# BrunoudA/MH-PPO

Measured on AMD Instinct MI355X. Metric: env-steps/sec at 65536 envs × 4 agents, 1/2/4/8 MI355X + %HBM roofline, higher is better.
Workload: dtype f64 env / f32 nets; 1 GPU; config 3: 4cars nb_car=4 nb_ped=1 nb_lines=2, 65536 envs/GPU x 80 steps, full PPO iteration (rollout + returns + 10+10 epochs); envs_per_gpu=65536, agents=4, T=80, parallelism=dp1

## Files before the change

### include/mhppo.h

```cpp
#ifndef MHPPO_H
#define MHPPO_H
#include <stdint.h>

#ifdef __cplusplus
extern "C" {
#endif

#define MHPPO_OK 0
#define MHPPO_EINVAL -1
#define MHPPO_EHIP -2
#define MHPPO_ENOMEM -3
#define MHPPO_ENAN -4

#define MHPPO_COOP 0
#define MHPPO_4CARS 1
#define MHPPO_SCALABLE 2
#define MHPPO_NAIF 3
#define MHPPO_4CARS2 4
#define MHPPO_STOP 5
#define MHPPO_FIX_SCALABLE_LANES 1
#define MHPPO_GENERIC_STEP 2

typedef struct mhppo_env_cfg {
    int32_t variant;
// ... 91 lines not shown
int mhppo_rollout_policy(mhppo_env *env, const mhppo_mlp *actor_cross, const mhppo_mlp *actor_wait,
                         mhppo_rollout_bufs *bufs, void *stream);
int mhppo_rollout_sample_env(mhppo_env *env, const float *eps, int t, mhppo_rollout_bufs *bufs, void *stream);
int mhppo_rollout_policy_part(mhppo_env *env, const mhppo_mlp *actor_cross, const mhppo_mlp *actor_wait,
                              mhppo_rollout_bufs *bufs, int part, void *stream);
int mhppo_rollout_sample_env_part(mhppo_env *env, const float *eps, int t, mhppo_rollout_bufs *bufs, int part,
                                  void *stream);

int mhppo_kernel_timing_begin(int n);
int mhppo_kernel_timing_end(double *ms_total, int *launches);
int mhppo_kernel_timing_end_each(float *ms_each, int cap, int *launches);

int mhppo_rollout_check(mhppo_rollout_bufs *bufs, void *stream);

int mhppo_philox_normal(uint64_t seed, uint64_t offset, float *out, int64_t n, void *stream);
int mhppo_philox_uniform(uint64_t seed, uint64_t offset, float *out, int64_t n, void *stream);
int mhppo_philox_normal_2d(uint64_t seed, uint64_t offset, uint64_t stride, float *out, int64_t rows,
                           int64_t cols, void *stream);


int mhppo_libm_eval(int fn, uint64_t first, int64_t n, float *out, void *stream);

int mhppo_returns_scan(const double *rew, float *ret, int64_t B, int32_t T, double gamma, void *stream);
int mhppo_returns_scan_tm(const double *rew, float *ret, int64_t B, int32_t T, double gamma, void *stream);

typedef struct {
  float *obs, *act, *logp, *ret;
  double *rew;
} mhppo_bucket_dst;
int mhppo_bucket_scatter(const int64_t *pos, const int8_t *bucket, int64_t NS, int32_t T, const float *obs_tm,
                         const float *act_tm, const float *logp_tm, const float *ret_tm, const double *rew_tm,
                         const mhppo_bucket_dst *dst, void *stream);

int mhppo_adv_stats(const float *ret, const float *value, int64_t M, double *stats, void *stream);
int mhppo_adv_normalize(const float *ret, const float *value, int64_t M, const double *stats,
                        double m_global, float *adv, void *stream);

int mhppo_ppo_cont_fwd_bwd(const float *mu, const float *act, const float *logp_old,
                           const float *adv, int64_t M, double inv_m, float *dmu,
                           double *loss, void *stream);

int mhppo_ppo_choice_fwd_bwd(const float *probs, const float *logp_old, const float *adv,
                             int64_t M, const double *counts, double inv_m2, float *dprobs,
                             double *loss, void *stream);

#define MHPPO_TRAIN_EXACT_F32 0x100
int mhppo_mlp_train(int kind, int n_in, const float *packed, const float *X, int64_t M, const float *ret,
                    float *value, const float *act, const float *logp_old, const double *stats,
                    const double *counts, double m_global, float out_mean, float out_std, float *grad,
                    double *sums, void *stream);

int mhppo_mlp_train_pair(const float *packed_actor, const float *packed_critic, const float *X, int64_t M,
                         const float *ret, float *value, const float *act, const float *logp_old,
                         const double *stats, double m_global, float out_mean, float out_std,
                         float *grad_actor, double *sums_actor, float *grad_critic, double *sums_critic,
                         void *stream);

int mhppo_mse_fwd_bwd(const float *value, const float *ret, int64_t M, double inv_m, float *dv,
                      double *loss, void *stream);

const char *mhppo_last_error(void);
const char *mhppo_version(void);

#ifdef __cplusplus
}
#endif
// ... 2 lines not shown
```

### mh-ppo_amd/csrc/rollout.hip

```cpp
#include <hip/hip_runtime.h>
#include <hip/hip_ext.h>

#include <vector>

#include <algorithm>
#include <math.h>
#include <string.h>

#include "../../include/mhppo.h"
#include "common.h"
#include "env_body.h"
#include "rollout_dev.h"
#include "libm_glibc.h"

using namespace mhppo;

namespace mhppo {
const Cfg &env_cfg(const mhppo_env *env);
const Bufs &env_bufs(const mhppo_env *env);
int env_device(const mhppo_env *env);
}

namespace {
constexpr int TPB = 256;
// ... 745 lines not shown
__global__ void __launch_bounds__(TPB) k_philox_normal_2d(uint64_t seed, uint64_t off, uint64_t stride, float *out,
                                                          int64_t rows, int64_t cols) {
  const int64_t i = (int64_t)blockIdx.x * TPB + threadIdx.x;
  if (i >= rows * cols) return;
  const int64_t r = i / cols, cc = i - r * cols;
  const uint64_t ctr = off + (uint64_t)r * stride + (uint64_t)cc;
  uint32_t c4[4] = {(uint32_t)ctr, (uint32_t)(ctr >> 32), 0x6d687070u, 0u};
  philox(c4, (uint32_t)seed, (uint32_t)(seed >> 32));
  const float u1 = ((float)(c4[0] >> 8) + 1.0f) * (1.0f / 16777216.0f);
  const float u2 = (float)(c4[1] >> 8) * (1.0f / 16777216.0f);
  out[i] = sqrtf(-2.0f * logf(u1)) * cosf(6.2831853071795865f * u2);
}

__global__ void __launch_bounds__(TPB) k_returns(const double *rew, float *ret, int64_t B, int T, double gamma) {
  int64_t b = (int64_t)blockIdx.x * TPB + threadIdx.x;
  if (b >= B) return;
  const double *r = rew + b * T;
  float *o = ret + b * T;
  double g = 0.0;
  for (int t = T - 1; t >= 0; t--) {
    g = r[t] + gamma * g;
    o[t] = (float)g;
  }
}

namespace bk {
constexpr int SEGS = 64, STEPS = 16;
constexpr int OBS_SEG = STEPS * NF_C + 1, V_SEG = STEPS + 1;
#ifndef MHPPO_BK_TPB
#define MHPPO_BK_TPB 1024
#endif
constexpr int BTPB = MHPPO_BK_TPB;
}
__global__ void __launch_bounds__(bk::BTPB)
    k_bucket_scatter(const int64_t *__restrict__ pos, const int8_t *__restrict__ bucket, int64_t NS, int T,
                     const float *__restrict__ obs, const float *__restrict__ act, const float *__restrict__ logp,
                     const float *__restrict__ ret, const double *__restrict__ rew, mhppo_bucket_dst d0,
                     mhppo_bucket_dst d1) {
  using namespace bk;
  __shared__ float s_obs[SEGS * OBS_SEG];
  __shared__ float s_v[3][SEGS * V_SEG];
  __shared__ double s_rew[SEGS * V_SEG];
  __shared__ int64_t s_pos[SEGS];
  __shared__ int8_t s_b[SEGS];
  const int64_t s0 = (int64_t)blockIdx.x * SEGS;
  const int t0 = blockIdx.y * STEPS;
  const int nseg = (int)min((int64_t)SEGS, NS - s0), nt = min(STEPS, T - t0);
  const int tid = threadIdx.x;
  if (tid < SEGS) {
    s_pos[tid] = tid < nseg ? pos[s0 + tid] : -1;
    s_b[tid] = tid < nseg ? bucket[s0 + tid] : 0;
  }
  __syncthreads();
  {
    constexpr int NQ = SEGS * NF_C * STEPS / BTPB;
    static_assert(SEGS * NF_C * STEPS % BTPB == 0, "bucket scatter: block size");
    float v[NQ];
    int at[NQ];
#pragma unroll
    for (int q = 0; q < NQ; q++) {
      const int i = tid + q * BTPB, tl = i / (SEGS * NF_C), k = i - tl * (SEGS * NF_C), sg = k / NF_C;
      const bool in = sg < nseg && tl < nt;
      at[q] = in && s_pos[sg] >= 0 ? sg * OBS_SEG + tl * NF_C + (k - sg * NF_C) : -1;
      v[q] = 0.0f;
      if (at[q] >= 0) v[q] = obs[((int64_t)(t0 + tl) * NS + s0) * NF_C + k];
    }
#pragma unroll
    for (int q = 0; q < NQ; q++)
      if (at[q] >= 0) s_obs[at[q]] = v[q];
  }
#pragma unroll
  for (int i = tid; i < SEGS * STEPS; i += BTPB) {
    const int sg = i % SEGS, tl = i / SEGS;
    if (sg >= nseg || tl >= nt || s_pos[sg] < 0) continue;
    const int64_t rec = (int64_t)(t0 + tl) * NS + s0 + sg;
    const int o = sg * V_SEG + tl;
    s_v[0][o] = act[rec];
    s_v[1][o] = logp[rec];
    s_v[2][o] = ret[rec];
    s_rew[o] = rew[rec];
  }
  __syncthreads();
  const int w = tid >> 6, l = tid & 63;
  for (int sg = w; sg < nseg; sg += BTPB / 64) {
    const int64_t p = s_pos[sg];
    if (p < 0) continue;
    const mhppo_bucket_dst &D = s_b[sg] ? d1 : d0;
    const int64_t r0 = p * T + t0;
    float *oo = D.obs + r0 * NF_C;
    for (int j = l; j < nt * NF_C; j += 64) oo[j] = s_obs[sg * OBS_SEG + j];
    if (l < nt) {
      const int o = sg * V_SEG + l;
      D.act[r0 + l] = s_v[0][o];
      D.logp[r0 + l] = s_v[1][o];
      D.ret[r0 + l] = s_v[2][o];
      D.rew[r0 + l] = s_rew[o];
    }
  }
}

__global__ void __launch_bounds__(TPB) k_returns_tm(const double *rew, float *ret, int64_t B, int T, double gamma) {
  int64_t b = (int64_t)blockIdx.x * TPB + threadIdx.x;
  if (b >= B) return;
  double g = 0.0;
  for (int t = T - 1; t >= 0; t--) {
    g = rew[(int64_t)t * B + b] + gamma * g;
    ret[(int64_t)t * B + b] = (float)g;
  }
}

template <int NP>
__device__ inline void block_reduce_store(double (&v)[NP], double *partials, int nblocks) {
  __shared__ double sh[NP][TPB];
#pragma unroll
  for (int k = 0; k < NP; k++) sh[k][threadIdx.x] = v[k];
  __syncthreads();
  for (int s = TPB / 2; s > 0; s >>= 1) {
    if ((int)threadIdx.x < s)
#pragma unroll
      for (int k = 0; k < NP; k++) sh[k][threadIdx.x] += sh[k][threadIdx.x + s];
    __syncthreads();
  }
  if (threadIdx.x == 0)
#pragma unroll
    for (int k = 0; k < NP; k++) partials[(size_t)k * nblocks + blockIdx.x] = sh[k][0];
}

__global__ void __launch_bounds__(TPB) k_sum_partials(const double *partials, int nblocks, int np, double *out) {
  __shared__ double sh[TPB];
  int k = blockIdx.x;
  double s = 0.0;
  for (int b = threadIdx.x; b < nblocks; b += TPB) s += partials[(size_t)k * nblocks + b];
  sh[threadIdx.x] = s;
  __syncthreads();
  for (int w = TPB / 2; w > 0; w >>= 1) {
    if ((int)threadIdx.x < w) sh[threadIdx.x] += sh[threadIdx.x + w];
    __syncthreads();
  }
  if (threadIdx.x == 0) out[k] += sh[0];
}

__global__ void __launch_bounds__(TPB) k_adv_stats(const float *ret, const float *val, int64_t M, double *partials) {
  int64_t i = (int64_t)blockIdx.x * TPB + threadIdx.x;
  double v[2] = {0.0, 0.0};
  if (i < M) {
    float a = ret[i] - val[i];
    v[0] = a;
    v[1] = (double)a * (double)a;
  }
  block_reduce_store<2>(v, partials, gridDim.x);
}

__global__ void __launch_bounds__(TPB)
    k_adv_norm(const float *ret, const float *val, int64_t M, const double *stats, double mg, float *adv) {
  int64_t i = (int64_t)blockIdx.x * TPB + threadIdx.x;
  if (i >= M) return;
  double mean = stats[0] / mg;
  double var = (stats[1] - stats[0] * mean) / (mg - 1.0);
  float meanf = (float)mean, stdf = (float)sqrt(var > 0 ? var : 0.0);
  float a = ret[i] - val[i];
  adv[i] = (a - meanf) / (stdf + 1e-10f);
}

__global__ void __launch_bounds__(TPB)
    k_ppo_cont(const float *mu, const float *act, const float *lp_old, const float *adv, int64_t M, double inv_m,
               float *dmu, double *partials) {
  int64_t i = (int64_t)blockIdx.x * TPB + threadIdx.x;
  double v[1] = {0.0};
  if (i < M) {
    float diff = (float)((double)act[i] - (double)mu[i]);
    float x = diff * MVN_INV_L;
    float lp = (-0.5f * (MVN_LOG2PI + x * x)) - MVN_HALF_LOGDET;
// ... 444 lines not shown
  if (!out || n < 0 || fn < 0 || fn > 2) return set_error(MHPPO_EINVAL, "bad argument (fn 0 tanhf, 1 expm1f, 2 expf)");
  if (n == 0) return MHPPO_OK;
  hipLaunchKernelGGL(k_libm_eval, grid_for(n), dim3(TPB), 0, (hipStream_t)stream, fn, first, n, out);
  CHECK_HIP(hipGetLastError());
  return MHPPO_OK;
}

int mhppo_returns_scan(const double *rew, float *ret, int64_t B, int32_t T, double gamma, void *stream) {
  if (!rew || !ret || B < 0 || T <= 0) return set_error(MHPPO_EINVAL, "bad argument");
  if (B == 0) return MHPPO_OK;
  hipLaunchKernelGGL(k_returns, grid_for(B), dim3(TPB), 0, (hipStream_t)stream, rew, ret, B, T, gamma);
  CHECK_HIP(hipGetLastError());
  return MHPPO_OK;
}

int mhppo_returns_scan_tm(const double *rew, float *ret, int64_t B, int32_t T, double gamma, void *stream) {
  if (!rew || !ret || B < 0 || T <= 0) return set_error(MHPPO_EINVAL, "bad argument");
  if (B == 0) return MHPPO_OK;
  hipLaunchKernelGGL(k_returns_tm, grid_for(B), dim3(TPB), 0, (hipStream_t)stream, rew, ret, B, T, gamma);
  CHECK_HIP(hipGetLastError());
  return MHPPO_OK;
}

int mhppo_bucket_scatter(const int64_t *pos, const int8_t *bucket, int64_t NS, int32_t T, const float *obs_tm,
                         const float *act_tm, const float *logp_tm, const float *ret_tm, const double *rew_tm,
                         const mhppo_bucket_dst *dst, void *stream) {
  if (NS < 0 || T <= 0 || !dst) return set_error(MHPPO_EINVAL, "bad argument");
  if (NS == 0) return MHPPO_OK;
  if (!pos || !bucket || !obs_tm || !act_tm || !logp_tm || !ret_tm || !rew_tm)
    return set_error(MHPPO_EINVAL, "null pointer");
  const int64_t nb = (NS + bk::SEGS - 1) / bk::SEGS;
  if (nb > 0x7fffffff) return set_error(MHPPO_EINVAL, "too many segments");
  dim3 g((unsigned)nb, (unsigned)((T + bk::STEPS - 1) / bk::STEPS));
  hipLaunchKernelGGL(k_bucket_scatter, g, dim3(bk::BTPB), 0, (hipStream_t)stream, pos, bucket, NS, (int)T, obs_tm,
                     act_tm, logp_tm, ret_tm, rew_tm, dst[0], dst[1]);
  CHECK_HIP(hipGetLastError());
  return MHPPO_OK;
}

int mhppo_adv_stats(const float *ret, const float *value, int64_t M, double *stats, void *stream) {
  if (M == 0) return MHPPO_OK;
  if (!ret || !value || !stats || M < 0) return set_error(MHPPO_EINVAL, "bad argument");
  dim3 g = grid_for(M);
  double *part = scratch(2 * (size_t)g.x);
  if (!part) return set_error(MHPPO_ENOMEM, "scratch allocation failed");
  hipStream_t s = (hipStream_t)stream;
  hipLaunchKernelGGL(k_adv_stats, g, dim3(TPB), 0, s, ret, value, M, part);
  hipLaunchKernelGGL(k_sum_partials, dim3(2), dim3(TPB), 0, s, part, (int)g.x, 2, stats);
  CHECK_HIP(hipGetLastError());
  return MHPPO_OK;
}

int mhppo_adv_normalize(const float *ret, const float *value, int64_t M, const double *stats, double m_global,
                        float *adv, void *stream) {
  if (M == 0) return MHPPO_OK;
  if (!ret || !value || !stats || !adv || M < 0) return set_error(MHPPO_EINVAL, "bad argument");
  hipLaunchKernelGGL(k_adv_norm, grid_for(M), dim3(TPB), 0, (hipStream_t)stream, ret, value, M, stats, m_global,
                     adv);
  CHECK_HIP(hipGetLastError());
  return MHPPO_OK;
}

int mhppo_ppo_cont_fwd_bwd(const float *mu, const float *act, const float *logp_old, const float *adv, int64_t M,
                           double inv_m, float *dmu, double *loss, void *stream) {
  if (M == 0) return MHPPO_OK;
  if (!mu || !act || !logp_old || !adv || !dmu || !loss || M < 0) return set_error(MHPPO_EINVAL, "bad argument");
  dim3 g = grid_for(M);
  double *part = scratch(g.x);
// ... 39 lines not shown
```

### mh-ppo_amd/mhppo/_lib.py

```python
import ctypes
import os

HERE = os.path.dirname(os.path.abspath(__file__))
LIB_PATH = os.environ.get("MHPPO_LIB") or os.path.join(HERE, "lib", "libmhppo.so")

P = ctypes.c_void_p
I32 = ctypes.c_int32
I64 = ctypes.c_int64
U64 = ctypes.c_uint64
F64 = ctypes.c_double


class EnvCfg(ctypes.Structure):
    _fields_ = [
        ("variant", I32), ("n_envs", I32), ("nb_car", I32), ("nb_ped", I32), ("nb_lines", I32),
        ("max_episode", I32), ("sin_model", I32), ("flags", I32), ("dt", F64),
        ("car_b", F64 * 4), ("ped_b", F64 * 8), ("cross_b", F64 * 2), ("seed_base", U64),
        ("env_id_offset", U64),
    ]


class Mlp(ctypes.Structure):
    _fields_ = [("packed", P), ("n_in", I32), ("n_out", I32), ("kind", I32), ("reserved", I32),
                ("mean", ctypes.c_float), ("std", ctypes.c_float)]
# ... 23 lines not shown
    "mhppo_env_reward_slots": (I32, [P]),
    "mhppo_env_state_dim": (I32, [P]),
    "mhppo_env_reset": (I32, [P, P, P]),
    "mhppo_env_choix_test": (I32, [P, P, P]),
    "mhppo_env_state_bytes": (I64, [P]),
    "mhppo_env_export": (I32, [P, P, P]),
    "mhppo_env_import": (I32, [P, P, P]),
    "mhppo_env_step": (I32, [P, P, P, P, P, P, P]),
    "mhppo_env_get_state": (I32, [P, P, P]),
    "mhppo_env_get_rng": (I32, [P, P, P, P]),
    "mhppo_env_events": (I32, [P, P, P]),
    "mhppo_choice_dim": (I32, [P]),
    "mhppo_rollout_begin": (I32, [P, ctypes.POINTER(Mlp), P, P, ctypes.POINTER(RolloutBufs), P]),
    "mhppo_rollout_step": (I32, [P, ctypes.POINTER(Mlp), ctypes.POINTER(Mlp), P, I32,
                                 ctypes.POINTER(RolloutBufs), P]),
    "mhppo_rollout_policy": (I32, [P, ctypes.POINTER(Mlp), ctypes.POINTER(Mlp), ctypes.POINTER(RolloutBufs), P]),
    "mhppo_rollout_sample_env": (I32, [P, P, I32, ctypes.POINTER(RolloutBufs), P]),
    "mhppo_rollout_policy_part": (I32, [P, ctypes.POINTER(Mlp), ctypes.POINTER(Mlp), ctypes.POINTER(RolloutBufs), I32,
                                        P]),
    "mhppo_rollout_sample_env_part": (I32, [P, P, I32, ctypes.POINTER(RolloutBufs), I32, P]),
    "mhppo_kernel_timing_begin": (I32, [I32]),
    "mhppo_kernel_timing_end": (I32, [ctypes.POINTER(ctypes.c_double), ctypes.POINTER(I32)]),
    "mhppo_kernel_timing_end_each": (I32, [P, I32, ctypes.POINTER(I32)]),
    "mhppo_eval_step": (I32, [P, ctypes.POINTER(Mlp), ctypes.POINTER(Mlp), ctypes.POINTER(Mlp), I32,
                              ctypes.POINTER(EvalBufs), P]),
    "mhppo_rollout_check": (I32, [ctypes.POINTER(RolloutBufs), P]),
    "mhppo_philox_normal": (I32, [U64, U64, P, I64, P]),
    "mhppo_philox_uniform": (I32, [U64, U64, P, I64, P]),
    "mhppo_philox_normal_2d": (I32, [U64, U64, U64, P, I64, I64, P]),
    "mhppo_libm_eval": (I32, [I32, U64, I64, P, P]),
    "mhppo_returns_scan": (I32, [P, P, I64, I32, F64, P]),
    "mhppo_returns_scan_tm": (I32, [P, P, I64, I32, F64, P]),
    "mhppo_bucket_scatter": (I32, [P, P, I64, I32] + [P] * 7),
    "mhppo_adv_stats": (I32, [P, P, I64, P, P]),
    "mhppo_adv_normalize": (I32, [P, P, I64, P, F64, P, P]),
    "mhppo_ppo_cont_fwd_bwd": (I32, [P, P, P, P, I64, F64, P, P, P]),
    "mhppo_ppo_choice_fwd_bwd": (I32, [P, P, P, I64, P, F64, P, P, P]),
    "mhppo_mse_fwd_bwd": (I32, [P, P, I64, F64, P, P, P]),
    "mhppo_mlp_train": (I32, [I32, I32, P, P, I64, P, P, P, P, P, P, F64, ctypes.c_float, ctypes.c_float, P, P, P]),
    "mhppo_mlp_train_pair": (I32, [P, P, P, I64, P, P, P, P, P, F64, ctypes.c_float, ctypes.c_float, P, P, P, P, P]),
    "mhppo_last_error": (ctypes.c_char_p, []),
    "mhppo_version": (ctypes.c_char_p, []),
}

_lib = None


class MhppoError(RuntimeError):
    pass


class MhppoNaNError(MhppoError, ValueError):
    """MHPPO_ENAN: a NaN policy output was sampled (the reference raises ValueError there)."""

ENAN = -4


def lib():
    global _lib
    if _lib is None:
        if not os.path.exists(LIB_PATH):
            raise MhppoError(f"{LIB_PATH} is missing: build it with `python -c 'import __graft_entry__ as g; g.build()'`")
        L = ctypes.CDLL(LIB_PATH)
        for name, (res, args) in _SIGS.items():
            fn = getattr(L, name)
            fn.restype = res
# ... 27 lines not shown
```

### mh-ppo_amd/mhppo/algo.py

```python
import contextlib
import os

import numpy as np
import torch
import torch.distributed as dist

from . import _lib, ppo
from .env import VecCrosswalk
from .models import Model_PPO
from .rollout import RolloutGPU, bucket_segments

PREFIX = {"scalable": "pappo-scalable-coop", "coop": "pappo-coop", "4cars": "pappo-coop-4cars", "naif": "pappo-acc6"}


def _rank():
    return dist.get_rank() if dist.is_available() and dist.is_initialized() else 0


def _rank_path(path):
    if dist.is_available() and dist.is_initialized() and dist.get_world_size() > 1:
        return f"{path}.rank{dist.get_rank()}"
    return path


# ... 163 lines not shown
            if m_d > 0:
                heads.append(ppo.Head("d", self.actor_net_choice, self.critic_net_choice, self.optimizer_actor_choice,
                                      self.optimizer_critic_choice, d["obs"], d["act"], d["logp"], d["ret"], m_d,
                                      counts, per_row=self.fix_choice_loss, exact=self.exact_f32))
                names.append("choice")
            losses = ppo.train_epochs(heads, 10, self.grad_bucket) if heads else None
        if self.verbose and losses is not None:
            div = {"cross": (m_c, m_c), "wait": (m_w, m_w), "choice": (m_d * m_d, m_d)}
            if self.fix_choice_loss:
                div["choice"] = (m_d, m_d)
            self.last_losses = {k: (float(a.item()) / div[k][0], float(b.item()) / div[k][1])
                                for k, (a, b) in zip(names, losses)}
        return m_c, m_w, m_d

    def evaluate(self, nbr_episodes, choix=False):
        self.rollout.reset()
        return self.rollout.iterations(self.actor_net_cross, self.actor_net_wait, self.actor_net_choice,
                                       nbr_episodes, choix=choix)

    def get_average(self, states):
        from .stats import get_average
        v = self.venv
        return get_average(states, v.variant, v.nb_car, v.nb_ped, v.nb_lines)

    def train(self, nb_loop, replay=None):
        self.rollout.fix_bucket = self.fix_bucket
        for ep in range(nb_loop):
            self.rollout.reset()
            fc, et = replay[ep] if replay is not None else (None, None)
            self.rollout.iterations_rand(self.actor_net_cross, self.actor_net_wait, self.actor_net_choice,
                                         self.cov_mat, self.cov_mat_d, self.batch_size, forced_choice=fc,
                                         eps_tape=et)
            m_c, m_w, m_d = self.update()
            rc, rw, rd = self.rollout.immediate_rewards()
            dev = self.venv.device
            sums = torch.stack([rc.double().sum(), rw.double().sum(), rd.double().sum()]).to(dev)
            ppo._allreduce_(sums)
            if dev.type == "cuda":
                host = torch.empty(3, dtype=torch.float64, pin_memory=True)
                host.copy_(sums, non_blocking=True)
                ev = torch.cuda.Event()
                ev.record(torch.cuda.current_stream(dev))
                self._pending_curves.append((host, ev, m_c, m_w, m_d))
            else:
                self._pending_curves.append((sums.clone(), None, m_c, m_w, m_d))
            if self.verbose:
                self._flush_curves()
            if self.verbose and _rank() == 0:
                print("Episode * {} * And Number of steps is ==> {}".format(ep, ep * self.batch_size))
                print("Average Cross reward is ==> {}, Average Wait reward is ==> {}".format(
                    np.mean(self.ep_reward_cross[-10:]) if self.ep_reward_cross else float("nan"),
                    np.mean(self.ep_reward_wait[-10:]) if self.ep_reward_wait else float("nan")))
                print("Average Choice reward is ==> {}".format(np.mean(self.ep_reward_choice[-10:])))
                print("Number Cross is ==> {} and Number Wait is ==> {} ".format(int(m_c), int(m_w)))
            self.rollout.reset()
            self.total_loop = self.total_loop + 1
            if len(self._pending_curves) > 1:
                self._flush_curves(keep_last=True)
        self._flush_curves()
        if _rank() == 0 and self.save_curves:
            self.save_reward_curves()
        if self.verbose and _rank() == 0:
            print("Complete")

    def _flush_curves(self, keep_last=False):
        n = len(self._pending_curves) - (1 if keep_last else 0)
        for host, ev, m_c, m_w, m_d in self._pending_curves[:n]:
            if ev is not None:
                ev.synchronize()
# ... 91 lines not shown
```

### mh-ppo_amd/mhppo/ppo.py

```python
import contextlib
import os

import torch
import torch.distributed as dist

from . import _lib


_FORCE_COLLECTIVES = False


def set_force_collectives(flag=True):
    global _FORCE_COLLECTIVES
    _FORCE_COLLECTIVES = bool(flag)


def _dp():
    if not (dist.is_available() and dist.is_initialized()):
        return False
    return _FORCE_COLLECTIVES or dist.get_world_size() > 1


def _allreduce_(t):
    if _dp():
# ... 293 lines not shown
def _actor_pass(p, h, stats, sums, st):
    ev = _ev_begin()
    _lib.check(_lib.lib().mhppo_mlp_train(
        p.akind | p.flags, p.n_in, p.wa, p.obs.data_ptr(), p.M, p.ret.data_ptr(), p.V.data_ptr(),
        None if p.act is None else p.act.data_ptr(), p.lp.data_ptr(), stats.data_ptr(),
        None if p.counts is None else p.counts.data_ptr(), h.m, p.mean, p.std, p.ga, sums.data_ptr(), st))
    _ev_end(ev, p.akind, p.n_in, p.M)


def _pair_pass(p, h, stats, sums_a, sums_c, st):
    ev = _ev_begin()
    _lib.check(_lib.lib().mhppo_mlp_train_pair(
        p.wa, p.wc, p.obs.data_ptr(), p.M, p.ret.data_ptr(), p.V.data_ptr(), p.act.data_ptr(), p.lp.data_ptr(),
        stats.data_ptr(), h.m, p.mean, p.std, p.ga, sums_a.data_ptr(), p.gc, sums_c.data_ptr(), st))
    _ev_end(ev, 3, 13, p.M)


TRAIN_STREAMS = max(1, int(os.environ.get("MHPPO_TRAIN_STREAMS", "1")))
_SIDE_STREAMS = {}


def _side_streams(dev, n):
    if dev.type != "cuda" or n <= 0:
        return []
    key = (dev.index if dev.index is not None else torch.cuda.current_device(), n)
    if key not in _SIDE_STREAMS:
        _SIDE_STREAMS[key] = [torch.cuda.Stream(device=dev) for _ in range(n)]
    return _SIDE_STREAMS[key]


def train_epochs(heads, n_epochs, bucket=None):
    H = len(heads)
    dev = heads[0].obs.device
    paired = [_use_pair(h) for h in heads]
    plans = [_HeadPlan(h) if h.obs.shape[0] > 0 else None for h in heads]
    main = torch.cuda.current_stream(dev) if dev.type == "cuda" else None
    side = _side_streams(dev, min(TRAIN_STREAMS, H) - 1)
    streams = [main] + side
    stats = None
    out = [[None, None] for _ in range(H)]
    for k in range(n_epochs + 1):
        sums = torch.zeros(2 * H, 3, dtype=torch.float64, device=dev)
        crit = k < n_epochs
        trained = []
        if side:
            fork = torch.cuda.Event()
            fork.record(main)
            for sd in side:
                sd.wait_event(fork)
        for i, h in enumerate(heads):
            p = plans[i]
            sc, sa = sums[i], sums[H + i]
            sti = streams[i % len(streams)]
            ctx = torch.cuda.stream(sti) if sti is not None else contextlib.nullcontext()
            st = sti.cuda_stream if sti is not None else None
            with ctx:
                stp = stats[2 * i:2 * i + 2] if k > 0 else None
                if p is None:
                    if k > 0:
                        cont = h.kind == "c"
                        k_mlp_train(KIND_CONT if cont else KIND_CHOICE, h.actor, h.obs, h.ret, h.obs.new_empty(0),
                                    h.act if (cont or h.per_row) else None, h.logp, stp,
                                    None if (cont or h.per_row) else h.counts, m_global=h.m, sums=sa, exact=h.exact)
                        trained.append(h.actor)
                        out[i][0] = sums[H + i, 0:1]
                    if crit:
                        k_mlp_train(KIND_CRITIC, h.critic, h.obs, h.ret, m_global=h.m, sums=sc, exact=h.exact)
                        trained.append(h.critic)
                        out[i][1] = sums[i, 0:1]
                    continue
                if k > 0 and crit and paired[i]:
                    _pair_pass(p, h, stp, sa, sc, st)
                    trained += [h.actor, h.critic]
                    out[i] = [sums[H + i, 0:1], sums[i, 0:1]]
                    continue
                if k > 0:
                    _actor_pass(p, h, stp, sa, st)
                    trained.append(h.actor)
                    out[i][0] = sums[H + i, 0:1]
                if crit:
                    _critic_pass(p, h, sc, st)
                    trained.append(h.critic)
                    out[i][1] = sums[i, 0:1]
        for sd in side:
            main.wait_stream(sd)
        if crit:
            stats = sums[:H, 1:3].reshape(-1).contiguous()
            _allreduce_(stats)
        if bucket is not None:
            bucket.allreduce(trained)
        else:
            _allreduce_net_grads(*trained)
        adam_steps([h.opt_actor for h in heads if h.actor in trained] +
                   [h.opt_critic for h in heads if h.critic in trained])
    del plans
    return [tuple(o) for o in out]


def _no_step_hooks(o):
    from torch.optim import optimizer as _opt
    return not (getattr(o, "_optimizer_step_pre_hooks", None) or getattr(o, "_optimizer_step_post_hooks", None)
                or getattr(_opt, "_global_optimizer_pre_hooks", None)
                or getattr(_opt, "_global_optimizer_post_hooks", None))


def _fused_adam_ok(o):
    return (hasattr(torch, "_fused_adam_") and hasattr(torch, "_foreach_add_") and _no_step_hooks(o)
            and isinstance(o, torch.optim.Adam) and getattr(o, "grad_scale", None) is None
            and getattr(o, "found_inf", None) is None
            and all(g.get("fused") and not g.get("amsgrad") and not g.get("capturable") and not g.get("differentiable")
                    and not g.get("decoupled_weight_decay", False) and not isinstance(g["lr"], torch.Tensor)
                    for g in o.param_groups))


class _AdamPlan:

    def __init__(self, opts, keys, groups, steps, grads):
        self.opts, self.keys, self.groups, self.steps = opts, keys, groups, steps
        self.refs = [(o.state, o.param_groups) for o in opts]
# ... 82 lines not shown
```

### mh-ppo_amd/mhppo/rollout.py

```python
import ctypes
import os

import torch

from . import _lib

NF_C = 13
_CTR_STEP = 1 << 40


class RolloutBatch:

    _REC = ("obs_c", "act", "logp", "rew")

    def __init__(self, **kw):
        self.__dict__.update(kw)

    def __getattr__(self, name):
        if name not in RolloutBatch._REC or self.__dict__.get("rec_of") is None:
            raise AttributeError(name)
        N, S, T = self.N, self.S, self.T
        ro = self.rec_of.long()
        x = getattr(self, name + "_tm").reshape(T, N * S, -1).index_select(1, ro.clamp_min(0))
        x = torch.where((ro >= 0).reshape(1, -1, 1), x, torch.zeros((), dtype=x.dtype, device=x.device))
# ... 204 lines not shown

def returns_scan_tm(rew_tm, gamma=0.99):
    T = rew_tm.shape[0]
    r = rew_tm.reshape(T, -1).contiguous()
    out = torch.empty(r.shape, dtype=torch.float32, device=rew_tm.device)
    with torch.cuda.device(rew_tm.device):
        _lib.check(_lib.lib().mhppo_returns_scan_tm(_lib.ptr(r), _lib.ptr(out), r.shape[1], T, gamma,
                                                    _lib.stream_ptr(device=rew_tm.device)))
    return out.reshape(rew_tm.shape)


def returns_scan(rew, gamma=0.99):
    T = rew.shape[-1]
    r = rew.reshape(-1, T).contiguous()
    out = torch.empty(r.shape, dtype=torch.float32, device=rew.device)
    with torch.cuda.device(rew.device):
        _lib.check(_lib.lib().mhppo_returns_scan(_lib.ptr(r), _lib.ptr(out), r.shape[0], T, gamma,
                                                 _lib.stream_ptr(device=rew.device)))
    return out.reshape(rew.shape)


NAN_STATUS_MSG = {1: "Categorical probs of the choice actor, :409",
                  2: "MultivariateNormal loc of the continuous actors, :451"}


def raise_if_nan_status(st):
    st = int(st)
    if st:
        what = "; ".join(m for b, m in NAN_STATUS_MSG.items() if st & b)
        raise _lib.MhppoNaNError(f"NaN policy output sampled ({what}): the reference raises ValueError here")


def bucket_segments(batch, fix_bucket=False, status=None):
    N, S, P, T = batch.N, batch.S, batch.P, batch.T
    a_flat = batch.a_d.reshape(N, S * P)
    if fix_bucket:
        a_car = batch.a_d.reshape(N, S, P).gather(2, batch.closest.reshape(N, S, 1).long()).reshape(N, S)
        action_d_i = 2 * a_car.to(torch.int32) - 1
    else:
        action_d_i = 2 * a_flat[:, :S].to(torch.int32) - 1
    exist = batch.exist.bool().reshape(-1)
    cross = exist & (action_d_i <= 0).reshape(-1)
    wait = exist & (action_d_i > 0).reshape(-1)
    NS = N * S
    ret = returns_scan_tm(batch.rew_tm)
    cc, cw = torch.cumsum(cross, 0), torch.cumsum(wait, 0)
    w0 = torch.div(cc[-1] + 3, 4, rounding_mode="floor") * 4
    pos = torch.where(cross, cc - 1, torch.where(wait, w0 + cw - 1, -1))
    bucket = torch.zeros(NS, dtype=torch.int8, device=pos.device)
    rec_of = getattr(batch, "rec_of", None)
    if rec_of is not None:
        idx = torch.where(rec_of >= 0, rec_of, NS).long()
        pos = torch.full((NS + 1,), -1, dtype=pos.dtype, device=pos.device).scatter_(0, idx, pos)[:NS]
    (both,) = scatter_positions(pos, bucket, (NS + 3,), NS, T, batch.obs_c_tm, batch.act_tm, batch.logp_tm, ret,
                                batch.rew_tm)
    seg_all = torch.nonzero_static(exist, size=NS, fill_value=0).squeeze(1)
    cl = batch.closest.reshape(NS).long().index_select(0, seg_all)
    base = seg_all * P + cl
    dc = batch.feat_d.shape[-1]
    a_sel = batch.a_d.reshape(-1).index_select(0, base)
    choice = dict(
        obs=batch.feat_d.reshape(NS * P, dc).index_select(0, base),
        act=a_sel,
        logp=batch.logp_d.reshape(-1).index_select(0, base),
        ret=batch.ep_min.reshape(-1).index_select(0, seg_all).float(),
    )
    a_car = batch.a_d.reshape(NS, P).gather(1, batch.closest.reshape(NS, 1).long()).reshape(-1)
    counts = torch.stack([(exist & (a_car == 0)).sum(), (exist & (a_car == 1)).sum()]).to(torch.float64)
    sizes = [cc[-1], cw[-1], exist.sum()]
    if status is not None:
        sizes.append(status.reshape(-1)[0].to(torch.int64))
    sizes = torch.stack(sizes).tolist()
    if status is not None:
        if sizes[3]:
            status.zero_()
        raise_if_nan_status(sizes[3])
    n_cross, n_wait, n_all = sizes[:3]
    c0 = (n_cross + 3) // 4 * 4
    cross_r = {k: both[k][:n_cross * T] for k in ("obs", "act", "logp", "ret", "rew")}
    wait_r = {k: both[k][c0 * T:(c0 + n_wait) * T] for k in ("obs", "act", "logp", "ret", "rew")}
    cross_r["n_seg"], wait_r["n_seg"] = n_cross, n_wait
    choice = {k: v[:n_all] for k, v in choice.items()}
    choice["n_seg"] = n_all
    choice["counts"] = counts
    return cross_r, wait_r, choice

# ... 28 lines not shown
```

Before: 75.61 million env-steps/s.

## Replace torch bucket planning with native count/scan/place kernels and fused reward sums

```diff
diff --git a/include/mhppo.h b/include/mhppo.h
--- a/include/mhppo.h
+++ b/include/mhppo.h
@@ -147,6 +147,22 @@
                          const float *act_tm, const float *logp_tm, const float *ret_tm, const double *rew_tm,
                          const mhppo_bucket_dst *dst, void *stream);
 
+int mhppo_bucket_scatter_sums(const int64_t *pos, const int8_t *bucket, int64_t NS, int32_t T, const float *obs_tm,
+                              const float *act_tm, const float *logp_tm, const float *ret_tm, const double *rew_tm,
+                              const mhppo_bucket_dst *dst, double *rew_sums, void *work, void *stream);
+
+typedef struct {
+  int64_t n_cross, n_wait, n_all, status;
+  double counts[2];
+  double rew_sums[3];
+} mhppo_bucket_info;
+int64_t mhppo_bucket_work_bytes(int64_t NS, int32_t T);
+int mhppo_bucket_plan(int64_t N, int32_t S, int32_t P, int32_t dc, const int32_t *a_d, const int32_t *closest,
+                      const uint8_t *exist, const int32_t *rec_of, const double *ep_min, const float *feat_d,
+                      const float *logp_d, int32_t fix_bucket, const int32_t *status, int64_t *pos, int8_t *bucket,
+                      float *c_obs, int32_t *c_act, float *c_logp, float *c_ret, mhppo_bucket_info *info,
+                      void *work, void *stream);
+
 int mhppo_adv_stats(const float *ret, const float *value, int64_t M, double *stats, void *stream);
 int mhppo_adv_normalize(const float *ret, const float *value, int64_t M, const double *stats,
                         double m_global, float *adv, void *stream);
diff --git a/mh-ppo_amd/csrc/rollout.hip b/mh-ppo_amd/csrc/rollout.hip
--- a/mh-ppo_amd/csrc/rollout.hip
+++ b/mh-ppo_amd/csrc/rollout.hip
@@ -801,17 +801,19 @@
 #endif
 constexpr int BTPB = MHPPO_BK_TPB;
 }
+template <bool SUMS>
 __global__ void __launch_bounds__(bk::BTPB)
     k_bucket_scatter(const int64_t *__restrict__ pos, const int8_t *__restrict__ bucket, int64_t NS, int T,
                      const float *__restrict__ obs, const float *__restrict__ act, const float *__restrict__ logp,
                      const float *__restrict__ ret, const double *__restrict__ rew, mhppo_bucket_dst d0,
-                     mhppo_bucket_dst d1) {
+                     mhppo_bucket_dst d1, double *__restrict__ partials) {
   using namespace bk;
   __shared__ float s_obs[SEGS * OBS_SEG];
   __shared__ float s_v[3][SEGS * V_SEG];
   __shared__ double s_rew[SEGS * V_SEG];
   __shared__ int64_t s_pos[SEGS];
   __shared__ int8_t s_b[SEGS];
+  __shared__ double s_sum[2][SUMS ? BTPB / 64 : 1];
   const int64_t s0 = (int64_t)blockIdx.x * SEGS;
   const int t0 = blockIdx.y * STEPS;
   const int nseg = (int)min((int64_t)SEGS, NS - s0), nt = min(STEPS, T - t0);
@@ -838,6 +840,7 @@
     for (int q = 0; q < NQ; q++)
       if (at[q] >= 0) s_obs[at[q]] = v[q];
   }
+  double acc[2] = {0.0, 0.0};
 #pragma unroll
   for (int i = tid; i < SEGS * STEPS; i += BTPB) {
     const int sg = i % SEGS, tl = i / SEGS;
@@ -847,9 +850,25 @@
     s_v[0][o] = act[rec];
     s_v[1][o] = logp[rec];
     s_v[2][o] = ret[rec];
-    s_rew[o] = rew[rec];
-  }
-  __syncthreads();
+    const double r = rew[rec];
+    s_rew[o] = r;
+    if (SUMS) acc[s_b[sg] ? 1 : 0] += (double)(float)r;
+  }
+  if (SUMS) {
+#pragma unroll
+    for (int k = 0; k < 2; k++) {
+      double a = acc[k];
+      for (int m = 32; m > 0; m >>= 1) a += __shfl_xor(a, m, 64);
+      if ((tid & 63) == 0) s_sum[k][tid >> 6] = a;
+    }
+  }
+  __syncthreads();
+  if (SUMS && tid < 2) {
+    double a = 0.0;
+    for (int q = 0; q < BTPB / 64; q++) a += s_sum[tid][q];
+    const size_t nblocks = (size_t)gridDim.x * gridDim.y;
+    partials[tid * nblocks + (size_t)blockIdx.y * gridDim.x + blockIdx.x] = a;
+  }
   const int w = tid >> 6, l = tid & 63;
   for (int sg = w; sg < nseg; sg += BTPB / 64) {
     const int64_t p = s_pos[sg];
@@ -878,6 +897,171 @@
   }
 }
 
+struct PlanSeg {
+  int64_t base;
+  int a_car;
+  bool exist, cross, wait;
+};
+__device__ inline PlanSeg plan_seg(int64_t s, int S, int P, const int32_t *__restrict__ a_d,
+                                   const int32_t *__restrict__ closest, const uint8_t *__restrict__ exist, int fix) {
+  PlanSeg q;
+  const int cl = min(max(closest[s], 0), P - 1);
+  q.base = s * P + cl;
+  q.a_car = a_d[q.base];
+  const int64_t n = s / S;
+  const int a = fix ? q.a_car : a_d[n * S * P + (s - n * S)];
+  q.exist = exist[s] != 0;
+  q.cross = q.exist && a <= 0;
+  q.wait = q.exist && a > 0;
+  return q;
+}
+
+constexpr int PLAN_NC = 5;
+
+__global__ void __launch_bounds__(TPB)
+    k_plan_count(int64_t NS, int S, int P, const int32_t *__restrict__ a_d, const int32_t *__restrict__ closest,
+                 const uint8_t *__restrict__ exist, const double *__restrict__ ep_min, int fix, int nblk,
+                 int32_t *__restrict__ cnt, double *__restrict__ epart, int64_t *__restrict__ pos,
+                 int8_t *__restrict__ bucket) {
+  __shared__ int wsum[PLAN_NC][TPB / 64];
+  __shared__ double sh[TPB];
+  const int64_t s = (int64_t)blockIdx.x * TPB + threadIdx.x;
+  bool f[PLAN_NC] = {false, false, false, false, false};
+  double e = 0.0;
+  if (s < NS) {
+    const PlanSeg q = plan_seg(s, S, P, a_d, closest, exist, fix);
+    f[0] = q.cross, f[1] = q.wait, f[2] = q.exist;
+    f[3] = q.exist && q.a_car == 0, f[4] = q.exist && q.a_car == 1;
+    if (q.exist) e = (double)(float)ep_min[s];
+    pos[s] = -1;
+    bucket[s] = 0;
+  }
+#pragma unroll
+  for (int k = 0; k < PLAN_NC; k++) {
+    const uint64_t m = __ballot(f[k]);
+    if ((threadIdx.x & 63) == 0) wsum[k][threadIdx.x >> 6] = __popcll(m);
+  }
+  sh[threadIdx.x] = e;
+  __syncthreads();
+  for (int st = TPB / 2; st > 0; st >>= 1) {
+    if ((int)threadIdx.x < st) sh[threadIdx.x] += sh[threadIdx.x + st];
+    __syncthreads();
+  }
+  if (threadIdx.x < PLAN_NC) {
+    int c = 0;
+    for (int w = 0; w < TPB / 64; w++) c += wsum[threadIdx.x][w];
+    cnt[(size_t)threadIdx.x * nblk + blockIdx.x] = c;
+  }
+  if (threadIdx.x == 0) epart[blockIdx.x] = sh[0];
+}
+
+__global__ void __launch_bounds__(TPB)
+    k_plan_scan(const int32_t *__restrict__ cnt, const double *__restrict__ epart, int nblk,
+                const int32_t *__restrict__ status, int32_t *__restrict__ base, mhppo_bucket_info *__restrict__ info) {
+  __shared__ int wsum[TPB / 64];
+  __shared__ double sh[TPB];
+  const int tid = threadIdx.x, lane = tid & 63, w = tid >> 6;
+  int64_t total[PLAN_NC];
+#pragma unroll
+  for (int k = 0; k < PLAN_NC; k++) {
+    int64_t carry = 0;
+    for (int b0 = 0; b0 < nblk; b0 += TPB) {
+      const int b = b0 + tid;
+      const int v = b < nblk ? cnt[(size_t)k * nblk + b] : 0;
+      int x = v;
+      for (int d = 1; d < 64; d <<= 1) {
+        const int y = __shfl_up(x, d, 64);
+        if (lane >= d) x += y;
+      }
+      if (lane == 63) wsum[w] = x;
+      __syncthreads();
+      int before = 0, all = 0;
+      for (int q = 0; q < TPB / 64; q++) {
+        if (q < w) before += wsum[q];
+        all += wsum[q];
+      }
+      if (k < 3 && b < nblk) base[(size_t)k * nblk + b] = (int32_t)(carry + before + x - v);
+      carry += all;
+      __syncthreads();
+    }
+    total[k] = carry;
+  }
+  double e = 0.0;
+  for (int b = tid; b < nblk; b += TPB) e += epart[b];
+  sh[tid] = e;
+  __syncthreads();
+  for (int st = TPB / 2; st > 0; st >>= 1) {
+    if (tid < st) sh[tid] += sh[tid + st];
+    __syncthreads();
+  }
+  if (tid == 0) {
+    info->n_cross = total[0];
+    info->n_wait = total[1];
+    info->n_all = total[2];
+    info->status = status ? status[0] : 0;
+    info->counts[0] = (double)total[3];
+    info->counts[1] = (double)total[4];
+    info->rew_sums[0] = 0.0;
+    info->rew_sums[1] = 0.0;
+    info->rew_sums[2] = sh[0];
+  }
+}
+
+__global__ void __launch_bounds__(TPB)
+    k_plan_place(int64_t NS, int S, int P, int dc, const int32_t *__restrict__ a_d,
+                 const int32_t *__restrict__ closest, const uint8_t *__restrict__ exist,
+                 const int32_t *__restrict__ rec_of, const double *__restrict__ ep_min,
+                 const float *__restrict__ feat_d, const float *__restrict__ logp_d, int fix, int nblk,
+                 const int32_t *__restrict__ base, const mhppo_bucket_info *__restrict__ info,
+                 int64_t *__restrict__ pos, int8_t *__restrict__ bucket, float *__restrict__ c_obs,
+                 int32_t *__restrict__ c_act, float *__restrict__ c_logp, float *__restrict__ c_ret) {
+  __shared__ int wsum[3][TPB / 64];
+  __shared__ int64_t s_src[TPB];
+  const int tid = threadIdx.x, lane = tid & 63, w = tid >> 6;
+  const int64_t s = (int64_t)blockIdx.x * TPB + tid;
+  PlanSeg q;
+  q.base = 0, q.a_car = 0, q.exist = q.cross = q.wait = false;
+  if (s < NS) q = plan_seg(s, S, P, a_d, closest, exist, fix);
+  const uint64_t mc = __ballot(q.cross), mw = __ballot(q.wait), me = __ballot(q.exist);
+  if (lane == 0) {
+    wsum[0][w] = __popcll(mc);
+    wsum[1][w] = __popcll(mw);
+    wsum[2][w] = __popcll(me);
+  }
+  __syncthreads();
+  int wc = 0, ww = 0, we = 0, ne = 0;
+  for (int k = 0; k < TPB / 64; k++) {
+    if (k < w) wc += wsum[0][k], ww += wsum[1][k], we += wsum[2][k];
+    ne += wsum[2][k];
+  }
+  const uint64_t lt = lane ? ((1ull << lane) - 1) : 0ull;
+  const int64_t ci = (int64_t)base[blockIdx.x] + wc + __popcll(mc & lt);
+  const int64_t wi = (int64_t)base[(size_t)nblk + blockIdx.x] + ww + __popcll(mw & lt);
+  const int er = we + __popcll(me & lt);
+  const int64_t eb = base[2 * (size_t)nblk + blockIdx.x];
+  const int64_t w0 = (info->n_cross + 3) / 4 * 4;
+  if (q.cross || q.wait) {
+    int64_t r = s;
+    if (rec_of) r = rec_of[s];
+    if (r >= 0 && r < NS) {
+      pos[r] = q.cross ? ci : w0 + wi;
+      bucket[r] = q.cross ? 0 : 1;
+    }
+  }
+  if (q.exist) {
+    s_src[er] = q.base;
+    c_act[eb + er] = q.a_car;
+    c_logp[eb + er] = logp_d[q.base];
+    c_ret[eb + er] = (float)ep_min[s];
+  }
+  __syncthreads();
+  float *o = c_obs + eb * dc;
+  for (int i = tid; i < ne * dc; i += TPB) {
+    const int r = i / dc, c = i - r * dc;
+    o[i] = feat_d[s_src[r] * dc + c];
+  }
+}
+
 template <int NP>
 __device__ inline void block_reduce_store(double (&v)[NP], double *partials, int nblocks) {
   __shared__ double sh[NP][TPB];
@@ -907,6 +1091,24 @@
     __syncthreads();
   }
   if (threadIdx.x == 0) out[k] += sh[0];
+}
+
+constexpr int FOLD_TPB = 1024;
+__global__ void __launch_bounds__(FOLD_TPB) k_sum_partials_wide(const double *partials, int nblocks, double *out) {
+  __shared__ double sh[FOLD_TPB];
+  const double *p = partials + (size_t)blockIdx.x * nblocks;
+  double a[4] = {0.0, 0.0, 0.0, 0.0};
+  for (int b = threadIdx.x; b < nblocks; b += 4 * FOLD_TPB)
+#pragma unroll
+    for (int u = 0; u < 4; u++)
+      if (b + u * FOLD_TPB < nblocks) a[u] += p[b + u * FOLD_TPB];
+  sh[threadIdx.x] = (a[0] + a[1]) + (a[2] + a[3]);
+  __syncthreads();
+  for (int w = FOLD_TPB / 2; w > 0; w >>= 1) {
+    if ((int)threadIdx.x < w) sh[threadIdx.x] += sh[threadIdx.x + w];
+    __syncthreads();
+  }
+  if (threadIdx.x == 0) out[blockIdx.x] += sh[0];
 }
 
 __global__ void __launch_bounds__(TPB) k_adv_stats(const float *ret, const float *val, int64_t M, double *partials) {
@@ -1417,8 +1619,65 @@
   const int64_t nb = (NS + bk::SEGS - 1) / bk::SEGS;
   if (nb > 0x7fffffff) return set_error(MHPPO_EINVAL, "too many segments");
   dim3 g((unsigned)nb, (unsigned)((T + bk::STEPS - 1) / bk::STEPS));
-  hipLaunchKernelGGL(k_bucket_scatter, g, dim3(bk::BTPB), 0, (hipStream_t)stream, pos, bucket, NS, (int)T, obs_tm,
-                     act_tm, logp_tm, ret_tm, rew_tm, dst[0], dst[1]);
+  hipLaunchKernelGGL(k_bucket_scatter<false>, g, dim3(bk::BTPB), 0, (hipStream_t)stream, pos, bucket, NS, (int)T,
+                     obs_tm, act_tm, logp_tm, ret_tm, rew_tm, dst[0], dst[1], (double *)nullptr);
+  CHECK_HIP(hipGetLastError());
+  return MHPPO_OK;
+}
+
+static int64_t plan_blocks(int64_t NS) { return (NS + TPB - 1) / TPB; }
+static int64_t scatter_blocks(int64_t NS, int32_t T) {
+  return ((NS + bk::SEGS - 1) / bk::SEGS) * ((T + bk::STEPS - 1) / bk::STEPS);
+}
+int64_t mhppo_bucket_work_bytes(int64_t NS, int32_t T) {
+  if (NS < 0 || T < 0) return 0;
+  const int64_t plan = plan_blocks(NS) * (8 + 4 * (PLAN_NC + 3)) + 8, sc = scatter_blocks(NS, T) * 16;
+  return std::max<int64_t>(std::max(plan, sc), 8);
+}
+
+int mhppo_bucket_scatter_sums(const int64_t *pos, const int8_t *bucket, int64_t NS, int32_t T, const float *obs_tm,
+                              const float *act_tm, const float *logp_tm, const float *ret_tm, const double *rew_tm,
+                              const mhppo_bucket_dst *dst, double *rew_sums, void *work, void *stream) {
+  if (NS < 0 || T <= 0 || !dst) return set_error(MHPPO_EINVAL, "bad argument");
+  if (NS == 0) return MHPPO_OK;
+  if (!pos || !bucket || !obs_tm || !act_tm || !logp_tm || !ret_tm || !rew_tm || !rew_sums || !work)
+    return set_error(MHPPO_EINVAL, "null pointer");
+  const int64_t nb = (NS + bk::SEGS - 1) / bk::SEGS, nblocks = scatter_blocks(NS, T);
+  if (nb > 0x7fffffff || nblocks > 0x7fffffff) return set_error(MHPPO_EINVAL, "too many segments");
+  dim3 g((unsigned)nb, (unsigned)((T + bk::STEPS - 1) / bk::STEPS));
+  hipStream_t s = (hipStream_t)stream;
+  double *part = (double *)work;
+  hipLaunchKernelGGL(k_bucket_scatter<true>, g, dim3(bk::BTPB), 0, s, pos, bucket, NS, (int)T, obs_tm, act_tm, logp_tm,
+                     ret_tm, rew_tm, dst[0], dst[1], part);
+  hipLaunchKernelGGL(k_sum_partials_wide, dim3(2), dim3(FOLD_TPB), 0, s, part, (int)nblocks, rew_sums);
+  CHECK_HIP(hipGetLastError());
+  return MHPPO_OK;
+}
+
+int mhppo_bucket_plan(int64_t N, int32_t S, int32_t P, int32_t dc, const int32_t *a_d, const int32_t *closest,
+                      const uint8_t *exist, const int32_t *rec_of, const double *ep_min, const float *feat_d,
+                      const float *logp_d, int32_t fix_bucket, const int32_t *status, int64_t *pos, int8_t *bucket,
+                      float *c_obs, int32_t *c_act, float *c_logp, float *c_ret, mhppo_bucket_info *info,
+                      void *work, void *stream) {
+  if (N < 0 || S <= 0 || P <= 0 || dc <= 0) return set_error(MHPPO_EINVAL, "bad argument");
+  if (!info || !work) return set_error(MHPPO_EINVAL, "null pointer");
+  const int64_t NS = N * S;
+  if (NS * P > 0x7fffffff) return set_error(MHPPO_EINVAL, "too many segments");
+  if (NS > 0 && (!a_d || !closest || !exist || !ep_min || !feat_d || !logp_d || !pos || !bucket || !c_obs || !c_act ||
+                 !c_logp || !c_ret))
+    return set_error(MHPPO_EINVAL, "null pointer");
+  const int nblk = (int)plan_blocks(NS);
+  double *epart = (double *)work;
+  int32_t *cnt = (int32_t *)(epart + nblk), *base = cnt + (size_t)PLAN_NC * nblk;
+  hipStream_t s = (hipStream_t)stream;
+  if (nblk > 0)
+    hipLaunchKernelGGL(k_plan_count, dim3(nblk), dim3(TPB), 0, s, NS, (int)S, (int)P, a_d, closest, exist, ep_min,
+                       (int)fix_bucket, nblk, cnt, epart, pos, bucket);
+  hipLaunchKernelGGL(k_plan_scan, dim3(1), dim3(TPB), 0, s, cnt, epart, nblk, status, base, info);
+  if (nblk > 0)
+    hipLaunchKernelGGL(k_plan_place, dim3(nblk), dim3(TPB), 0, s, NS, (int)S, (int)P, (int)dc, a_d, closest, exist,
+                       rec_of, ep_min, feat_d, logp_d, (int)fix_bucket, nblk, base, info, pos, bucket, c_obs, c_act,
+                       c_logp, c_ret);
   CHECK_HIP(hipGetLastError());
   return MHPPO_OK;
 }
diff --git a/mh-ppo_amd/mhppo/_lib.py b/mh-ppo_amd/mhppo/_lib.py
--- a/mh-ppo_amd/mhppo/_lib.py
+++ b/mh-ppo_amd/mhppo/_lib.py
@@ -79,6 +79,9 @@
     "mhppo_returns_scan": (I32, [P, P, I64, I32, F64, P]),
     "mhppo_returns_scan_tm": (I32, [P, P, I64, I32, F64, P]),
     "mhppo_bucket_scatter": (I32, [P, P, I64, I32] + [P] * 7),
+    "mhppo_bucket_scatter_sums": (I32, [P, P, I64, I32] + [P] * 9),
+    "mhppo_bucket_work_bytes": (I64, [I64, I32]),
+    "mhppo_bucket_plan": (I32, [I64, I32, I32, I32] + [P] * 7 + [I32] + [P] * 10),
     "mhppo_adv_stats": (I32, [P, P, I64, P, P]),
     "mhppo_adv_normalize": (I32, [P, P, I64, P, F64, P, P]),
     "mhppo_ppo_cont_fwd_bwd": (I32, [P, P, P, P, I64, F64, P, P, P]),
diff --git a/mh-ppo_amd/mhppo/algo.py b/mh-ppo_amd/mhppo/algo.py
--- a/mh-ppo_amd/mhppo/algo.py
+++ b/mh-ppo_amd/mhppo/algo.py
@@ -219,9 +219,13 @@
                                          self.cov_mat, self.cov_mat_d, self.batch_size, forced_choice=fc,
                                          eps_tape=et)
             m_c, m_w, m_d = self.update()
-            rc, rw, rd = self.rollout.immediate_rewards()
             dev = self.venv.device
-            sums = torch.stack([rc.double().sum(), rw.double().sum(), rd.double().sum()]).to(dev)
+            sums = (self.rollout.choice or {}).get("rew_sums")
+            if sums is None:
+                rc, rw, rd = self.rollout.immediate_rewards()
+                sums = torch.stack([rc.double().sum(), rw.double().sum(), rd.double().sum()]).to(dev)
+            elif ppo._dp():
+                sums = sums.clone()
             ppo._allreduce_(sums)
             if dev.type == "cuda":
                 host = torch.empty(3, dtype=torch.float64, pin_memory=True)
diff --git a/mh-ppo_amd/mhppo/ppo.py b/mh-ppo_amd/mhppo/ppo.py
--- a/mh-ppo_amd/mhppo/ppo.py
+++ b/mh-ppo_amd/mhppo/ppo.py
@@ -349,6 +349,8 @@
 def train_epochs(heads, n_epochs, bucket=None):
     H = len(heads)
     dev = heads[0].obs.device
+    all_sums = torch.zeros(n_epochs + 1, 2 * H, 3, dtype=torch.float64, device=dev)
+    dp = _dp()
     paired = [_use_pair(h) for h in heads]
     plans = [_HeadPlan(h) if h.obs.shape[0] > 0 else None for h in heads]
     main = torch.cuda.current_stream(dev) if dev.type == "cuda" else None
@@ -357,7 +359,7 @@
     stats = None
     out = [[None, None] for _ in range(H)]
     for k in range(n_epochs + 1):
-        sums = torch.zeros(2 * H, 3, dtype=torch.float64, device=dev)
+        sums = all_sums[k]
         crit = k < n_epochs
         trained = []
         if side:
@@ -372,7 +374,9 @@
             ctx = torch.cuda.stream(sti) if sti is not None else contextlib.nullcontext()
             st = sti.cuda_stream if sti is not None else None
             with ctx:
-                stp = stats[2 * i:2 * i + 2] if k > 0 else None
+                stp = None
+                if k > 0:
+                    stp = stats[2 * i:2 * i + 2] if dp else all_sums[k - 1, i, 1:3]
                 if p is None:
                     if k > 0:
                         cont = h.kind == "c"
@@ -401,7 +405,7 @@
                     out[i][1] = sums[i, 0:1]
         for sd in side:
             main.wait_stream(sd)
-        if crit:
+        if crit and dp:
             stats = sums[:H, 1:3].reshape(-1).contiguous()
             _allreduce_(stats)
         if bucket is not None:
diff --git a/mh-ppo_amd/mhppo/rollout.py b/mh-ppo_amd/mhppo/rollout.py
--- a/mh-ppo_amd/mhppo/rollout.py
+++ b/mh-ppo_amd/mhppo/rollout.py
@@ -260,6 +260,79 @@
 
 
 def bucket_segments(batch, fix_bucket=False, status=None):
+    if batch.a_d.device.type == "cuda":
+        return bucket_segments_native(batch, fix_bucket, status)
+    return bucket_segments_torch(batch, fix_bucket, status)
+
+
+def bucket_plan(batch, fix_bucket=False, status=None):
+    N, S, P, T = batch.N, batch.S, batch.P, batch.T
+    NS = N * S
+    dev = batch.a_d.device
+    L = _lib.lib()
+    dc = batch.feat_d.shape[-1]
+    e = lambda shape, dt: torch.empty(shape, dtype=dt, device=dev)
+    src = dict(a_d=batch.a_d.to(torch.int32), closest=batch.closest.to(torch.int32), exist=batch.exist.to(torch.uint8),
+               ep_min=batch.ep_min.to(torch.float64), feat_d=batch.feat_d.to(torch.float32),
+               logp_d=batch.logp_d.to(torch.float32))
+    src = {k: v.contiguous() for k, v in src.items()}
+    rec_of = getattr(batch, "rec_of", None)
+    if rec_of is not None:
+        rec_of = rec_of.to(torch.int32).contiguous()
+    out = dict(pos=e(NS, torch.int64), bucket=e(NS, torch.int8), obs=e((NS, dc), torch.float32),
+               act=e(NS, torch.int32), logp=e(NS, torch.float32), ret=e(NS, torch.float32), info=e(9, torch.int64),
+               work=e(max(1, int(L.mhppo_bucket_work_bytes(NS, T)) // 8), torch.float64))
+    p = _lib.ptr
+    with torch.cuda.device(dev):
+        _lib.check(L.mhppo_bucket_plan(N, S, P, dc, p(src["a_d"]), p(src["closest"]), p(src["exist"]), p(rec_of),
+                                       p(src["ep_min"]), p(src["feat_d"]), p(src["logp_d"]), int(bool(fix_bucket)),
+                                       p(status), p(out["pos"]), p(out["bucket"]), p(out["obs"]), p(out["act"]),
+                                       p(out["logp"]), p(out["ret"]), p(out["info"]), p(out["work"]),
+                                       _lib.stream_ptr(device=dev)))
+    return out
+
+
+def bucket_segments_native(batch, fix_bucket=False, status=None):
+    N, S, P, T = batch.N, batch.S, batch.P, batch.T
+    NS = N * S
+    dev = batch.a_d.device
+    L = _lib.lib()
+    ret_tm = returns_scan_tm(batch.rew_tm)
+    plan = bucket_plan(batch, fix_bucket, status)
+    info = plan["info"]
+    n = NS + 3
+    both = dict(obs=torch.empty(n * T, NF_C, dtype=torch.float32, device=dev),
+                act=torch.empty(n * T, dtype=torch.float32, device=dev),
+                logp=torch.empty(n * T, dtype=torch.float32, device=dev),
+                ret=torch.empty(n * T, dtype=torch.float32, device=dev),
+                rew=torch.empty(n * T, dtype=torch.float64, device=dev))
+    one = _lib.BucketDst(*[both[k].data_ptr() for k in ("obs", "act", "logp", "ret", "rew")])
+    dst = (_lib.BucketDst * 2)(one, one)
+    srcs = [x.contiguous() for x in (batch.obs_c_tm, batch.act_tm, batch.logp_tm)]
+    rew_tm = batch.rew_tm.contiguous()
+    p = _lib.ptr
+    args = (p(plan["pos"]), p(plan["bucket"]), NS, T, *[p(x) for x in srcs], p(ret_tm), p(rew_tm), dst,
+            ctypes.c_void_p(info.data_ptr() + 48), p(plan["work"]), _lib.stream_ptr(device=dev))
+    n_cross, n_wait, n_all, st = info[:4].tolist()
+    if status is not None:
+        if st:
+            status.zero_()
+        raise_if_nan_status(st)
+    with torch.cuda.device(dev):
+        _lib.check(L.mhppo_bucket_scatter_sums(*args))
+    c0 = (n_cross + 3) // 4 * 4
+    cross_r = {k: both[k][:n_cross * T] for k in ("obs", "act", "logp", "ret", "rew")}
+    wait_r = {k: both[k][c0 * T:(c0 + n_wait) * T] for k in ("obs", "act", "logp", "ret", "rew")}
+    cross_r["n_seg"], wait_r["n_seg"] = n_cross, n_wait
+    choice = {k: plan[k][:n_all] for k in ("obs", "act", "logp", "ret")}
+    choice["n_seg"] = n_all
+    f64 = info[4:9].view(torch.float64)
+    choice["counts"] = f64[0:2]
+    choice["rew_sums"] = f64[2:5]
+    return cross_r, wait_r, choice
+
+
+def bucket_segments_torch(batch, fix_bucket=False, status=None, plan_out=None):
     N, S, P, T = batch.N, batch.S, batch.P, batch.T
     a_flat = batch.a_d.reshape(N, S * P)
     if fix_bucket:
@@ -280,6 +353,8 @@
     if rec_of is not None:
         idx = torch.where(rec_of >= 0, rec_of, NS).long()
         pos = torch.full((NS + 1,), -1, dtype=pos.dtype, device=pos.device).scatter_(0, idx, pos)[:NS]
+    if plan_out is not None:
+        plan_out.update(pos=pos, wait=wait)
     (both,) = scatter_positions(pos, bucket, (NS + 3,), NS, T, batch.obs_c_tm, batch.act_tm, batch.logp_tm, ret,
                                 batch.rew_tm)
     seg_all = torch.nonzero_static(exist, size=NS, fill_value=0).squeeze(1)
```

New measurement: 77.01 million env-steps/s (median of 6 runs). +1.9%, better.
